# vllm-project/production-stack

Hardware: AMD Instinct MI355X
Metric: output_tokens_per_sec (higher is better)
Workload: dtype bfloat16; 1 GPU; multi-round-qa; model=llama-3-8b, users_per_gpu=320, rounds_per_conversation=10, max_model_len=8192, parallelism=dp1, prefix_caching=True, kv_cache_dtype=auto, quantization=none

## Files before the change

csrc/attention.hip:

```cpp
#include "ps_common.h"

template <int HEAD_DIM, int GQ, int BLOCK_SIZE, int NWAVES, int LOWREG,
          typename KVT>
__global__ __launch_bounds__(NWAVES * 64, LOWREG ? 3 : 1) void paged_attn_decode_kernel(
    unsigned short* __restrict__ out,
    float* __restrict__ ws_acc,
    float* __restrict__ ws_ml,
    const unsigned short* __restrict__ q,
    const KVT* __restrict__ k_cache,
    const KVT* __restrict__ v_cache,
    const int* __restrict__ block_tables,
    const int* __restrict__ seq_lens,
    int max_blocks, float scale, int KH, long q_stride, int window) {
  using KVTr = ps_kv_traits<KVT>;
  using kvec8 = typename KVTr::vec8;
  constexpr int D = HEAD_DIM;
  constexpr int LPG = D / 8;
  constexpr int TPW = 64 / LPG;
  static_assert(BLOCK_SIZE % TPW == 0, "block size must divide");

  const int seq = blockIdx.x;
  const int kvh = blockIdx.y;
  const int ctx = seq_lens[seq];
  const int wave = threadIdx.x >> 6;
  const int lane = threadIdx.x & 63;
  const int sg = lane / LPG;
  const int sl = lane % LPG;

  ps_bf16x8 qp[GQ];
  const unsigned short* qbase = q + (long)seq * q_stride + (long)kvh * GQ * D;
#pragma unroll
  for (int g = 0; g < GQ; g++)
    qp[g] = *(const ps_bf16x8*)(qbase + g * D + sl * 8);
  float qf[GQ][8];
  if constexpr (!LOWREG) {
#pragma unroll
    for (int g = 0; g < GQ; g++)
#pragma unroll
      for (int j = 0; j < 8; j++) qf[g][j] = ps_bf16_to_f32(qp[g][j]);
  }

  float m[GQ], l[GQ], acc[GQ][8];
#pragma unroll
  for (int g = 0; g < GQ; g++) {
    m[g] = PS_NEG_INF;
    l[g] = 0.f;
#pragma unroll
    for (int j = 0; j < 8; j++) acc[g][j] = 0.f;
  }

  const int nblocks = (ctx + BLOCK_SIZE - 1) / BLOCK_SIZE;
  const int win_lo = (window > 0 && ctx > window) ? ctx - window : 0;
  const int first_block = win_lo / BLOCK_SIZE;
  const int nsplit = gridDim.z;
  const int split = blockIdx.z;
  const int live_blocks = nblocks - first_block;
  const int per_split = (live_blocks + nsplit - 1) / nsplit;
  const int b_begin = first_block + split * per_split;
  const int b_end = min(nblocks, b_begin + per_split);
  const int* bt = block_tables + (long)seq * max_blocks;
  constexpr int TPB = BLOCK_SIZE / TPW;
  for (int b = b_begin + wave; b < b_end; b += NWAVES) {
    const long blk = bt[b];
    const KVT* kb = k_cache + ((blk * KH + kvh) * BLOCK_SIZE) * D;
    const KVT* vb = v_cache + ((blk * KH + kvh) * BLOCK_SIZE) * D;
    const int valid_tokens = min(BLOCK_SIZE, ctx - b * BLOCK_SIZE);
    float sc[GQ][TPB];
    kvec8 vv[TPB];
    if constexpr (LOWREG) {
#pragma unroll
      for (int g = 0; g < GQ; g++)
        asm volatile("" : "+v"(qp[g]));
    }
#pragma unroll
    for (int tt = 0; tt < TPB; tt++) {
      const int tok = tt * TPW + sg;
      const bool valid =
          tok < valid_tokens && b * BLOCK_SIZE + tok >= win_lo;
      kvec8 kv = *(const kvec8*)(kb + tok * D + sl * 8);
      if constexpr (!LOWREG)
        vv[tt] = *(const kvec8*)(vb + tok * D + sl * 8);
      float kf[8];
      KVTr::to_f32x8(kv, kf);
#pragma unroll
      for (int g = 0; g < GQ; g++) {
        float s = 0.f;
#pragma unroll
        for (int j = 0; j < 8; j++) {
          if constexpr (LOWREG)
            s += ps_bf16_to_f32(qp[g][j]) * kf[j];
          else
            s += qf[g][j] * kf[j];
        }
        s = ps_group_sum<LPG>(s) * scale;
        sc[g][tt] = valid ? s : PS_NEG_INF;
      }
    }
    if constexpr (LOWREG) {
#pragma unroll
      for (int tt = 0; tt < TPB; tt++)
        vv[tt] = *(const kvec8*)(vb + (tt * TPW + sg) * D + sl * 8);
    }
#pragma unroll
    for (int g = 0; g < GQ; g++) {
      float bmax = sc[g][0];
#pragma unroll
      for (int tt = 1; tt < TPB; tt++) bmax = fmaxf(bmax, sc[g][tt]);
      const float mnew = fmaxf(m[g], bmax);
      const float corr = __expf(m[g] - mnew);
      float p[TPB];
      float psum = 0.f;
#pragma unroll
      for (int tt = 0; tt < TPB; tt++) {
        p[tt] = sc[g][tt] > PS_NEG_INF ? __expf(sc[g][tt] - mnew) : 0.f;
        psum += p[tt];
// ... 32 lines not shown
  }

  __shared__ float sm[NWAVES][GQ];
  __shared__ float slse[NWAVES][GQ];
  __shared__ float sacc[NWAVES][GQ][D];
  if (sg == 0) {
#pragma unroll
    for (int g = 0; g < GQ; g++) {
      if (sl == 0) {
        sm[wave][g] = m[g];
        slse[wave][g] = l[g];
      }
#pragma unroll
      for (int j = 0; j < 8; j++) sacc[wave][g][sl * 8 + j] = acc[g][j];
    }
  }
  __syncthreads();
  if (wave == 0 && sg == 0) {
#pragma unroll
    for (int g = 0; g < GQ; g++) {
      float M = PS_NEG_INF, L = 0.f, A[8];
#pragma unroll
      for (int j = 0; j < 8; j++) A[j] = 0.f;
#pragma unroll
      for (int wv = 0; wv < NWAVES; wv++) {
        const float mw = sm[wv][g];
        const float mnew = fmaxf(M, mw);
        const float c1 = __expf(M - mnew);
        const float c2 = __expf(mw - mnew);
        L = L * c1 + slse[wv][g] * c2;
#pragma unroll
        for (int j = 0; j < 8; j++)
          A[j] = A[j] * c1 + sacc[wv][g][sl * 8 + j] * c2;
        M = mnew;
      }
      const long head = (long)seq * KH * GQ + (long)kvh * GQ + g;
      if (nsplit == 1) {
        const float inv = L > 0.f ? 1.f / L : 0.f;
        ps_bf16x8 ov;
#pragma unroll
        for (int j = 0; j < 8; j++) ov[j] = ps_f32_to_bf16(A[j] * inv);
        *(ps_bf16x8*)(out + head * D + sl * 8) = ov;
      } else {
        float* wa = ws_acc + (head * nsplit + split) * D + sl * 8;
#pragma unroll
        for (int j = 0; j < 8; j++) wa[j] = A[j];
        if (sl == 0) {
          float* wm = ws_ml + (head * nsplit + split) * 2;
          wm[0] = M;
          wm[1] = L;
        }
      }
    }
  }
}

template <int HEAD_DIM>
__global__ __launch_bounds__(64) void paged_attn_combine_kernel(
    unsigned short* __restrict__ out,
    const float* __restrict__ ws_acc,
    const float* __restrict__ ws_ml,
    int nsplit) {
  constexpr int D = HEAD_DIM;
  constexpr int LPG = D / 8;
  const long head = blockIdx.x;
  const int sl = threadIdx.x;
  if (sl >= LPG) return;
  float M = PS_NEG_INF, L = 0.f, A[8];
#pragma unroll
  for (int j = 0; j < 8; j++) A[j] = 0.f;
  for (int s = 0; s < nsplit; s++) {
    const float mw = ws_ml[(head * nsplit + s) * 2 + 0];
    const float lw = ws_ml[(head * nsplit + s) * 2 + 1];
    const float mnew = fmaxf(M, mw);
    const float c1 = __expf(M - mnew);
    const float c2 = __expf(mw - mnew);
    const float* wa = ws_acc + (head * nsplit + s) * D + sl * 8;
#pragma unroll
    for (int j = 0; j < 8; j++) A[j] = A[j] * c1 + wa[j] * c2;
    L = L * c1 + lw * c2;
    M = mnew;
  }
  const float inv = L > 0.f ? 1.f / L : 0.f;
  ps_bf16x8 ov;
#pragma unroll
  for (int j = 0; j < 8; j++) ov[j] = ps_f32_to_bf16(A[j] * inv);
  *(ps_bf16x8*)(out + head * D + sl * 8) = ov;
}

template <int HEAD_DIM, int BLOCK_SIZE>
__global__ __launch_bounds__(64) void paged_attn_prefill_kernel(
    unsigned short* __restrict__ out,
    const unsigned short* __restrict__ q,
    const unsigned short* __restrict__ k_cache,
    const unsigned short* __restrict__ v_cache,
    const int* __restrict__ block_tables,
    const int* __restrict__ token_seq,
    const int* __restrict__ token_pos,
    int max_blocks, float scale, int KH, int GQ, long q_stride,
    int window) {
  constexpr int D = HEAD_DIM;
  constexpr int LPG = D / 8;
  constexpr int TPW = 64 / LPG;

  const int tokid = blockIdx.x;
  const int qh = blockIdx.y;
// ... 123 lines not shown
    for (int j = 0; j < 8; j++) {
      const float f = ps_bf16_to_f32(xv[j]);
      if (f > best) {
        best = f;
        besti = i + j;
      }
    }
  }
  const int tail_start = (V / 8) * 8;
  for (int i = tail_start + threadIdx.x; i < V; i += blockDim.x) {
    const float f = ps_bf16_to_f32(row[i]);
    if (f > best) {
      best = f;
      besti = i;
    }
  }
#pragma unroll
  for (int off = 32; off > 0; off >>= 1) {
    const float ob = __shfl_xor(best, off, 64);
    const int oi = __shfl_xor(besti, off, 64);
    if (ob > best || (ob == best && oi < besti)) {
      best = ob;
      besti = oi;
    }
  }
  __shared__ float wbest[4];
  __shared__ int wbesti[4];
  const int wave = threadIdx.x >> 6;
  if ((threadIdx.x & 63) == 0) {
    wbest[wave] = best;
    wbesti[wave] = besti;
  }
  __syncthreads();
  if (threadIdx.x == 0) {
    for (int wv = 1; wv < (int)(blockDim.x >> 6); wv++) {
      if (wbest[wv] > wbest[0] ||
          (wbest[wv] == wbest[0] && wbesti[wv] < wbesti[0])) {
        wbest[0] = wbest[wv];
        wbesti[0] = wbesti[wv];
      }
    }
    out[r] = wbesti[0];
  }
}

extern "C" {

int ps_paged_attn_decode(void* out, void* ws_acc, void* ws_ml, const void* q,
                         const void* k_cache, const void* v_cache,
                         const void* block_tables, const void* seq_lens,
                         int num_seqs, int max_blocks, float scale, int KH,
                         int GQ, int head_dim, int block_size, int num_splits,
                         long q_stride, int variant, int kv_fp8,
                         int window, hipStream_t stream) {
  dim3 grid(num_seqs, KH, num_splits);
  constexpr int NW = 4;
  dim3 block(NW * 64);
#define PS_DECODE_T(HD, G, BS, LR, KVT)                                      \
  paged_attn_decode_kernel<HD, G, BS, NW, LR, KVT>                           \
      <<<grid, block, 0, stream>>>(                                          \
          (unsigned short*)out, (float*)ws_acc, (float*)ws_ml,               \
          (const unsigned short*)q, (const KVT*)k_cache,                     \
          (const KVT*)v_cache, (const int*)block_tables,                     \
          (const int*)seq_lens, max_blocks, scale, KH, q_stride, window)
#define PS_DISPATCH_DECODE(HD, G, BS)                                        \
  do {                                                                       \
    if (kv_fp8) {                                                            \
      if (variant == 1)                                                      \
        PS_DECODE_T(HD, G, BS, 1, unsigned char);                            \
      else                                                                   \
        PS_DECODE_T(HD, G, BS, 0, unsigned char);                            \
    } else {                                                                 \
      if (variant == 1)                                                      \
        PS_DECODE_T(HD, G, BS, 1, unsigned short);                           \
      else                                                                   \
        PS_DECODE_T(HD, G, BS, 0, unsigned short);                           \
    }                                                                        \
    if (num_splits > 1)                                                      \
      paged_attn_combine_kernel<HD>                                          \
          <<<dim3(num_seqs * KH * G), 64, 0, stream>>>(                      \
              (unsigned short*)out, (const float*)ws_acc,                    \
              (const float*)ws_ml, num_splits);                              \
  } while (0)
  if (head_dim == 128 && block_size == 16) {
    switch (GQ) {
      case 1: PS_DISPATCH_DECODE(128, 1, 16); return 0;
      case 2: PS_DISPATCH_DECODE(128, 2, 16); return 0;
      case 3: PS_DISPATCH_DECODE(128, 3, 16); return 0;
      case 4: PS_DISPATCH_DECODE(128, 4, 16); return 0;
      case 6: PS_DISPATCH_DECODE(128, 6, 16); return 0;
      case 7: PS_DISPATCH_DECODE(128, 7, 16); return 0;
      case 8: PS_DISPATCH_DECODE(128, 8, 16); return 0;
      default: return -1;
    }
  }
  if (head_dim == 64 && block_size == 16 && !kv_fp8) {
    switch (GQ) {
      case 1: PS_DISPATCH_DECODE(64, 1, 16); return 0;
      case 2: PS_DISPATCH_DECODE(64, 2, 16); return 0;
      case 4: PS_DISPATCH_DECODE(64, 4, 16); return 0;
      case 8: PS_DISPATCH_DECODE(64, 8, 16); return 0;
      default: return -1;
    }
  }
  return -1;
#undef PS_DECODE_T
#undef PS_DISPATCH_DECODE
}

int ps_paged_attn_prefill(void* out, const void* q, const void* k_cache,
                          const void* v_cache, const void* block_tables,
                          const void* token_seq, const void* token_pos,
                          int num_tokens, int num_q_heads, int max_blocks,
                          float scale, int KH, int GQ, int head_dim,
                          int block_size, long q_stride, int window,
                          hipStream_t stream) {
  dim3 grid(num_tokens, num_q_heads);
  dim3 block(64);
#define PS_DISPATCH_PREFILL(HD, BS)                                         \
  paged_attn_prefill_kernel<HD, BS><<<grid, block, 0, stream>>>(            \
      (unsigned short*)out, (const unsigned short*)q,                       \
      (const unsigned short*)k_cache, (const unsigned short*)v_cache,       \
      (const int*)block_tables, (const int*)token_seq,                      \
      (const int*)token_pos, max_blocks, scale, KH, GQ, q_stride, window)
  if (head_dim == 128 && block_size == 16) {
    PS_DISPATCH_PREFILL(128, 16);
    return 0;
  }
  if (head_dim == 64 && block_size == 16) {
    PS_DISPATCH_PREFILL(64, 16);
    return 0;
  }
  return -1;
#undef PS_DISPATCH_PREFILL
}

void ps_reshape_and_cache(const void* k, const void* v, void* k_cache,
                          void* v_cache, const void* slot_mapping, long T,
                          int KH, int HD, int BS, int kv_fp8,
                          hipStream_t stream) {
  const long total = T * (long)KH * HD / 8;
  const int block = 256;
  const long want = (total + block - 1) / block;
  const int grid = (int)(want < 2048 ? (want > 0 ? want : 1) : 2048);
  if (kv_fp8)
    reshape_and_cache_kernel<unsigned char><<<grid, block, 0, stream>>>(
        (const unsigned short*)k, (const unsigned short*)v,
        (unsigned char*)k_cache, (unsigned char*)v_cache,
        (const long*)slot_mapping, KH, HD, BS, total);
  else
    reshape_and_cache_kernel<unsigned short><<<grid, block, 0, stream>>>(
        (const unsigned short*)k, (const unsigned short*)v,
        (unsigned short*)k_cache, (unsigned short*)v_cache,
        (const long*)slot_mapping, KH, HD, BS, total);
}

void ps_greedy_sample(void* out, const void* logits, long R, int V,
                      hipStream_t stream) {
  greedy_sample_kernel<<<dim3((unsigned)R), 256, 0, stream>>>(
      (long*)out, (const unsigned short*)logits, V);
// ... 4 lines not shown
```

csrc/bindings.cpp:

```cpp
#include <hip/hip_runtime.h>
#include <torch/extension.h>

#include <c10/hip/HIPStream.h>

#include <algorithm>

extern "C" {
void ps_rms_norm(void* out, const void* x, const void* w, float eps, long T,
                 int D, hipStream_t stream);
void ps_fused_add_rms_norm(void* x, void* residual, const void* w, float eps,
                           long T, int D, hipStream_t stream);
void ps_rms_norm_fp8(void* out_q, void* out_scale, void* x, void* residual,
                     const void* w, float eps, long T, int D, int fused,
                     hipStream_t stream);
void ps_silu_and_mul_fp8(void* out_q, void* out_scale, const void* x, long T,
                         int D, hipStream_t stream);
void ps_silu_and_mul(void* out, const void* x, long T, int D,
                     hipStream_t stream);
void ps_rope(const void* positions, void* q, void* k, const void* cos_sin,
             long T, int QH, int KH, int HD, int ROT, hipStream_t stream);
void ps_fused_rope_cache(void* qkv, const void* positions, const void* cos_sin,
                         const void* slot_mapping, void* k_cache,
                         void* v_cache, long T, int QH, int KH, int HD,
                         int ROT, long qkv_stride, int BS, int kv_fp8,
                         hipStream_t stream);
int ps_paged_attn_decode(void* out, void* ws_acc, void* ws_ml, const void* q,
                         const void* k_cache, const void* v_cache,
                         const void* block_tables, const void* seq_lens,
                         int num_seqs, int max_blocks, float scale, int KH,
                         int GQ, int head_dim, int block_size, int num_splits,
                         long q_stride, int variant, int kv_fp8, int window,
                         hipStream_t stream);
int ps_prefill_mfma32_splits(int num_tiles, int KH, int GQ);
int ps_paged_attn_prefill_mfma32(void* out, void* ws_o, void* ws_ml,
                                 long q_tokens, const void* q,
                                 const void* k_cache, const void* v_cache,
                                 const void* block_tables,
                                 const void* tile_info, int num_tiles,
                                 int num_q_heads, int max_blocks,
                                 float scale, int KH, int GQ, int head_dim,
                                 long q_stride, int kv_fp8, int window,
                                 hipStream_t stream);
int ps_paged_attn_prefill_mfma(void* out, const void* q, const void* k_cache,
                               const void* v_cache, const void* block_tables,
                               const void* tile_info, int num_tiles,
                               int num_q_heads, int max_blocks, float scale,
                               int KH, int GQ, int head_dim, long q_stride,
                               int variant, int kv_fp8, int window, hipStream_t stream);
int ps_paged_attn_prefill(void* out, const void* q, const void* k_cache,
                          const void* v_cache, const void* block_tables,
                          const void* token_seq, const void* token_pos,
                          int num_tokens, int num_q_heads, int max_blocks,
                          float scale, int KH, int GQ, int head_dim,
                          int block_size, long q_stride, int window,
                          hipStream_t stream);
void ps_reshape_and_cache(const void* k, const void* v, void* k_cache,
                          void* v_cache, const void* slot_mapping, long T,
                          int KH, int HD, int BS, int kv_fp8,
                          hipStream_t stream);
void ps_greedy_sample(void* out, const void* logits, long R, int V,
                      hipStream_t stream);
void ps_kv_quant(void* out, void* scales, const void* in, long rows, int hd,
                 hipStream_t stream);
void ps_kv_dequant(void* out, const void* in, const void* scales, long rows,
                   int hd, hipStream_t stream);
int ps_skinny_gemm_splits(int M, int N, int K);
int ps_skinny_gemm(void* out_bf16, void* ws, const void* x, const void* w,
                   int M, int N, int K, long x_stride, hipStream_t stream);
int ps_gemm8p_splits(int M, int N, int K);
int ps_gemm8p(void* out_bf16, void* ws, const void* x, const void* w, int M,
              int N, int K, long x_stride, hipStream_t stream);
int ps_lora_bgmv(void* out, const void* x, const void* A, const void* B,
                 const void* scale, const void* idx, int T, int IN, int W,
                 int R, long out_stride, long x_stride, int col_off,
                 hipStream_t stream);
int ps_fused_moe_supported(int T, int top_k, int E, int H, int I);
int ps_fused_moe(void* out, void* offsets, void* sorted_pairs, void* act,
                 void* y, const void* x, const void* w_gate_up,
                 const void* w_down, const void* topk_ids, int ids_i64,
                 const void* topk_w, int T, int top_k, int E, int H, int I,
                 hipStream_t stream);
}

at::Tensor cachegen_encode(at::Tensor q);
at::Tensor cachegen_decode(at::Tensor blob, int64_t hd);
// ... 31 lines not shown
}

void rms_norm(at::Tensor out, at::Tensor x, at::Tensor w, double eps) {
  CHECK_GPU_BF16(out);
  CHECK_GPU_BF16(x);
  CHECK_GPU_BF16(w);
  const long T = x.numel() / x.size(-1);
  const int D = (int)x.size(-1);
  TORCH_CHECK(D % 8 == 0, "hidden dim must be a multiple of 8");
  ps_rms_norm(out.data_ptr(), x.data_ptr(), w.data_ptr(), (float)eps, T, D,
              current_stream());
}

void fused_add_rms_norm(at::Tensor x, at::Tensor residual, at::Tensor w,
                        double eps) {
  CHECK_GPU_BF16(x);
  CHECK_GPU_BF16(residual);
  CHECK_GPU_BF16(w);
  const long T = x.numel() / x.size(-1);
  const int D = (int)x.size(-1);
  TORCH_CHECK(D % 8 == 0, "hidden dim must be a multiple of 8");
  ps_fused_add_rms_norm(x.data_ptr(), residual.data_ptr(), w.data_ptr(),
                        (float)eps, T, D, current_stream());
}

void silu_and_mul(at::Tensor out, at::Tensor x) {
  CHECK_GPU_BF16(out);
  CHECK_GPU_BF16(x);
  const int D = (int)out.size(-1);
  TORCH_CHECK(x.size(-1) == 2 * D, "x last dim must be 2*out last dim");
  TORCH_CHECK(D % 8 == 0, "feature dim must be a multiple of 8");
  const long T = out.numel() / D;
  ps_silu_and_mul(out.data_ptr(), x.data_ptr(), T, D, current_stream());
}

void rotary_embedding(at::Tensor positions, at::Tensor q, at::Tensor k,
                      at::Tensor cos_sin, long head_dim) {
  CHECK_GPU_DTYPE(positions, at::kInt);
  CHECK_GPU_BF16(q);
  CHECK_GPU_BF16(k);
  CHECK_GPU_DTYPE(cos_sin, at::kFloat);
  const long T = positions.size(0);
  const int HD = (int)head_dim;
  const int ROT = (int)cos_sin.size(-1);
  const int QH = (int)(q.numel() / T / HD);
  const int KH = (int)(k.numel() / T / HD);
  ps_rope(positions.data_ptr(), q.data_ptr(), k.data_ptr(),
          cos_sin.data_ptr(), T, QH, KH, HD, ROT, current_stream());
}

void paged_attn_decode(at::Tensor out, at::Tensor q, at::Tensor k_cache,
                       at::Tensor v_cache, at::Tensor block_tables,
                       at::Tensor seq_lens, double scale, int64_t num_splits,
                       int64_t variant, int64_t window) {
  CHECK_GPU_BF16(out);
  const int kv_fp8 = cache_fp8(k_cache);
  cache_fp8(v_cache);
  CHECK_GPU_DTYPE(block_tables, at::kInt);
  CHECK_GPU_DTYPE(seq_lens, at::kInt);
  const int S = (int)q.size(0);
  const int QH = (int)q.size(1);
  const int HD = (int)q.size(2);
  const int KH = (int)k_cache.size(1);
  const int BS = (int)k_cache.size(2);
  TORCH_CHECK(QH % KH == 0, "GQA group mismatch");
  const int GQ = QH / KH;
  const int max_blocks = (int)block_tables.size(1);
  if (num_splits <= 0) {
    const int target = 2048;
    num_splits = std::min<int64_t>(
        32, std::max<int64_t>(1, target / std::max(1, S * KH)));
  }
  at::Tensor ws_acc, ws_ml;
  void *acc_p = nullptr, *ml_p = nullptr;
  if (num_splits > 1) {
    auto opts = q.options().dtype(at::kFloat);
    ws_acc = at::empty({(long)S * QH * num_splits * HD}, opts);
    ws_ml = at::empty({(long)S * QH * num_splits * 2}, opts);
    acc_p = ws_acc.data_ptr();
    ml_p = ws_ml.data_ptr();
  }
  int rc = ps_paged_attn_decode(
      out.data_ptr(), acc_p, ml_p, q.data_ptr(), k_cache.data_ptr(),
      v_cache.data_ptr(), block_tables.data_ptr(), seq_lens.data_ptr(), S,
      max_blocks, (float)scale, KH, GQ, HD, BS, (int)num_splits,
      q_row_stride(q, HD), (int)variant, kv_fp8, (int)window,
      current_stream());
  TORCH_CHECK(rc == 0, "unsupported decode config: head_dim=", HD,
              " block_size=", BS, " gqa=", GQ);
}

void paged_attn_prefill(at::Tensor out, at::Tensor q, at::Tensor k_cache,
                        at::Tensor v_cache, at::Tensor block_tables,
                        at::Tensor token_seq, at::Tensor token_pos,
                        double scale, int64_t window) {
  CHECK_GPU_BF16(out);
  CHECK_GPU_BF16(k_cache);
  CHECK_GPU_BF16(v_cache);
  CHECK_GPU_DTYPE(block_tables, at::kInt);
  CHECK_GPU_DTYPE(token_seq, at::kInt);
  CHECK_GPU_DTYPE(token_pos, at::kInt);
  const int T = (int)q.size(0);
  const int QH = (int)q.size(1);
  const int HD = (int)q.size(2);
  const int KH = (int)k_cache.size(1);
  const int BS = (int)k_cache.size(2);
  TORCH_CHECK(QH % KH == 0, "GQA group mismatch");
  const int GQ = QH / KH;
  const int max_blocks = (int)block_tables.size(1);
  int rc = ps_paged_attn_prefill(
      out.data_ptr(), q.data_ptr(), k_cache.data_ptr(), v_cache.data_ptr(),
      block_tables.data_ptr(), token_seq.data_ptr(), token_pos.data_ptr(), T,
      QH, max_blocks, (float)scale, KH, GQ, HD, BS, q_row_stride(q, HD),
      (int)window, current_stream());
  TORCH_CHECK(rc == 0, "unsupported prefill config: head_dim=", HD,
              " block_size=", BS);
}

void paged_attn_prefill_mfma(at::Tensor out, at::Tensor q,
                             at::Tensor k_cache, at::Tensor v_cache,
                             at::Tensor block_tables, at::Tensor tile_info,
                             double scale, int64_t variant, int64_t window) {
  CHECK_GPU_BF16(out);
  const int kv_fp8 = cache_fp8(k_cache);
  cache_fp8(v_cache);
  CHECK_GPU_DTYPE(block_tables, at::kInt);
  CHECK_GPU_DTYPE(tile_info, at::kInt);
  const int QH = (int)q.size(1);
  const int HD = (int)q.size(2);
  const int KH = (int)k_cache.size(1);
  TORCH_CHECK(QH % KH == 0, "GQA group mismatch");
  TORCH_CHECK(k_cache.size(2) == 16, "mfma prefill needs block_size 16");
  const int GQ = QH / KH;
  const int NT = (int)tile_info.size(0);
  int rc;
  if (variant == 5) {
    const int splits = ps_prefill_mfma32_splits(NT, KH, QH / KH);
    const long T = q.size(0);
    void *ws_o_p = nullptr, *ws_ml_p = nullptr;
    at::Tensor ws_o, ws_ml;
    if (splits > 1) {
      ws_o = at::empty({(long)splits * T * QH * HD},
// ... 214 lines not shown
  int rc = ps_fused_moe(
      out.data_ptr(), offsets.data_ptr(), sorted_pairs.data_ptr(),
      act.data_ptr(), y.data_ptr(), x.data_ptr(), experts_gate_up.data_ptr(),
      experts_down.data_ptr(), topk_ids.data_ptr(),
      topk_ids.scalar_type() == at::kLong ? 1 : 0, topk_w.data_ptr(), (int)T,
      (int)top_k, (int)E, (int)H, (int)I, current_stream());
  TORCH_CHECK(rc == 0, "fused_moe launch rejected");
}

void kv_quant(at::Tensor out, at::Tensor scales, at::Tensor in) {
  CHECK_GPU_DTYPE(out, at::kChar);
  CHECK_GPU_DTYPE(scales, at::kFloat);
  CHECK_GPU_BF16(in);
  const int hd = (int)in.size(-1);
  TORCH_CHECK(hd % 8 == 0, "row width must be multiple of 8");
  const long rows = in.numel() / hd;
  ps_kv_quant(out.data_ptr(), scales.data_ptr(), in.data_ptr(), rows, hd,
              current_stream());
}

void kv_dequant(at::Tensor out, at::Tensor in, at::Tensor scales) {
  CHECK_GPU_BF16(out);
  CHECK_GPU_DTYPE(in, at::kChar);
  CHECK_GPU_DTYPE(scales, at::kFloat);
  const int hd = (int)out.size(-1);
  const long rows = out.numel() / hd;
  ps_kv_dequant(out.data_ptr(), in.data_ptr(), scales.data_ptr(), rows, hd,
                current_stream());
}

void greedy_sample(at::Tensor out, at::Tensor logits) {
  CHECK_GPU_DTYPE(out, at::kLong);
  CHECK_GPU_BF16(logits);
  const long R = logits.size(0);
  const int V = (int)logits.size(1);
  ps_greedy_sample(out.data_ptr(), logits.data_ptr(), R, V, current_stream());
}

}

PYBIND11_MODULE(TORCH_EXTENSION_NAME, m) {
  m.def("rms_norm", &rms_norm, "RMSNorm (bf16)");
  m.def("fused_add_rms_norm", &fused_add_rms_norm,
        "Fused residual add + RMSNorm (bf16, in-place)");
  m.def("silu_and_mul", &silu_and_mul, "SiLU-and-mul (bf16)");
  m.def("rotary_embedding", &rotary_embedding,
        "Neox-style rotary embedding (bf16, in-place)");
  m.def("paged_attn_decode", &paged_attn_decode,
        "Paged attention, decode phase (bf16 KV, split-KV)",
        pybind11::arg("out"), pybind11::arg("q"), pybind11::arg("k_cache"),
        pybind11::arg("v_cache"), pybind11::arg("block_tables"),
        pybind11::arg("seq_lens"), pybind11::arg("scale"),
        pybind11::arg("num_splits") = 0, pybind11::arg("variant") = 0,
        pybind11::arg("window") = 0);
  m.def("paged_attn_prefill", &paged_attn_prefill,
        "Paged attention, chunked prefill (bf16 KV)");
  m.def("lora_bgmv", &lora_bgmv,
        "batched-grouped LoRA matvec (per-token adapter slots)");
  m.def("paged_attn_prefill_mfma", &paged_attn_prefill_mfma,
        "Paged attention, chunked prefill via MFMA tiles (head_dim 128)",
        pybind11::arg("out"), pybind11::arg("q"), pybind11::arg("k_cache"),
        pybind11::arg("v_cache"), pybind11::arg("block_tables"),
        pybind11::arg("tile_info"), pybind11::arg("scale"),
        pybind11::arg("variant") = 4, pybind11::arg("window") = 0);
  m.def("fused_rope_cache", &fused_rope_cache,
        "Fused RoPE + paged KV append on the packed qkv tensor");
  m.def("reshape_and_cache", &reshape_and_cache,
        "Append K/V for new tokens into the paged cache");
  m.def("greedy_sample", &greedy_sample, "Per-row argmax over vocab");
  m.def("kv_quant", &kv_quant, "Row-wise int8 KV quantization");
  m.def("rms_norm_fp8", &rms_norm_fp8,
        "RMSNorm (optionally fused residual add) emitting fp8 + row scales");
  m.def("silu_and_mul_fp8", &silu_and_mul_fp8,
        "SiLU-mul emitting fp8 + row scales");
  m.def("cachegen_encode", &cachegen_encode,
        "CacheGen-style adaptive range encode of int8 KV (CPU)");
  m.def("cachegen_decode", &cachegen_decode,
        "CacheGen-style range decode -> int8 (CPU)");
  m.def("gemm8p", &gemm8p,
        "8-phase deep-pipelined bf16 GEMM (out = x @ w.T)");
  m.def("skinny_gemm", &skinny_gemm,
        "Split-K MFMA GEMM for decode-shaped (M<=128) projections");
  m.def("gemm8p_splits", &ps_gemm8p_splits,
        "Split-K depth gemm8p picks for (M, N, K); -1 if unsupported");
  m.def("skinny_gemm_splits", &ps_skinny_gemm_splits,
        "Split-K depth skinny_gemm picks for (M, N, K); -1 if unsupported");
  m.def("kv_dequant", &kv_dequant, "Row-wise int8 KV dequantization");
  m.def("fused_moe", &fused_moe,
        "Grouped MoE expert MLP (align + gate_up/SiLU + down + combine)");
  m.def("fused_moe_supported", &fused_moe_supported,
        "Whether fused_moe accepts (T, top_k, E, H, I)");
}
```

production_stack_amd/engine/models/llama.py:

```python

from __future__ import annotations

import math
from typing import List, Optional

import torch
import torch.nn as nn
import torch.nn.functional as F

from production_stack_amd import ops
from production_stack_amd.ops import gemm_policy
from production_stack_amd.engine.config import ModelConfig
from production_stack_amd.parallel import state as pstate


class BatchMeta:

    def __init__(
        self,
        positions: torch.Tensor,
        slot_mapping: torch.Tensor,
        num_prefill_tokens: int,
        prefill_token_seq: Optional[torch.Tensor],
        prefill_token_pos: Optional[torch.Tensor],
        prefill_block_tables: Optional[torch.Tensor],
        num_decode_seqs: int,
        decode_seq_lens: Optional[torch.Tensor],
        decode_block_tables: Optional[torch.Tensor],
        prefill_tiles: Optional[torch.Tensor] = None,
        lora_groups=None,
        lora_idx: Optional[torch.Tensor] = None,
        mm_rows: Optional[torch.Tensor] = None,
        mm_embeds: Optional[torch.Tensor] = None,
    ) -> None:
        self.positions = positions
        self.slot_mapping = slot_mapping
        self.num_prefill_tokens = num_prefill_tokens
        self.prefill_token_seq = prefill_token_seq
        self.prefill_token_pos = prefill_token_pos
        self.prefill_block_tables = prefill_block_tables
        self.num_decode_seqs = num_decode_seqs
        self.decode_seq_lens = decode_seq_lens
        self.decode_block_tables = decode_block_tables
        self.prefill_tiles = prefill_tiles
        self.lora_groups = lora_groups or []
        self.lora_idx = lora_idx
        self.mm_rows = mm_rows
        self.mm_embeds = mm_embeds


def build_cos_sin_cache(
    head_dim: int, max_position: int, theta: float,
    rope_scaling=None,
) -> torch.Tensor:
    half = head_dim // 2
    inv = 1.0 / (
        theta ** (torch.arange(0, head_dim, 2, dtype=torch.float64) / head_dim)
    )
    if rope_scaling is not None:
        factor, low_f, high_f, orig_max = rope_scaling
        low_wl = orig_max / low_f
        high_wl = orig_max / high_f
        wavelen = 2 * math.pi / inv
        scaled = torch.where(wavelen > low_wl, inv / factor, inv)
        smooth = (orig_max / wavelen - low_f) / (high_f - low_f)
        mid = (1 - smooth) * (inv / factor) + smooth * inv
        in_band = (wavelen <= low_wl) & (wavelen >= high_wl)
        inv = torch.where(in_band, mid, scaled)
    t = torch.arange(max_position, dtype=torch.float64)
    freqs = torch.outer(t, inv)
    return torch.cat([freqs.cos(), freqs.sin()], dim=-1).float().contiguous()


class LlamaLayer(nn.Module):
    def __init__(self, cfg: ModelConfig, tp: int, layer_idx: int = 0) -> None:
        super().__init__()
        self.cfg = cfg
        self.layer_idx = layer_idx
        assert cfg.num_q_heads % tp == 0, "q heads must divide TP"
        assert cfg.num_kv_heads % tp == 0 or tp % cfg.num_kv_heads == 0
        self.q_heads = cfg.num_q_heads // tp
        self.kv_heads = max(cfg.num_kv_heads // tp, 1)
        self.head_dim = cfg.head_dim
        self.inter = cfg.intermediate_size // tp
        h = cfg.hidden_size
        qs = self.q_heads * self.head_dim
        kvs = self.kv_heads * self.head_dim
        self.qkv_proj = nn.Parameter(
            torch.empty(qs + 2 * kvs, h, dtype=torch.bfloat16)
        )
        self.o_proj = nn.Parameter(torch.empty(h, qs, dtype=torch.bfloat16))
        self.n_experts = cfg.num_experts
        self.top_k = cfg.num_experts_per_tok
        self.moe_backend = "loop"
        if self.n_experts:
            self.moe_gate = nn.Parameter(
                torch.empty(self.n_experts, h, dtype=torch.bfloat16)
            )
            self.experts_gate_up = nn.Parameter(
                torch.empty(self.n_experts, 2 * self.inter, h,
                            dtype=torch.bfloat16)
# ... 90 lines not shown
            q, k = ops.rotary_embedding(
                meta.positions, q, k, cos_sin, self.head_dim
            )
            ops.reshape_and_cache(
                k.view(T, self.kv_heads, self.head_dim),
                v.view(T, self.kv_heads, self.head_dim),
                k_cache,
                v_cache,
                meta.slot_mapping,
            )
            qh = q.view(T, self.q_heads, self.head_dim)
        outs: List[torch.Tensor] = []
        tp = meta.num_prefill_tokens
        if tp > 0:
            if (
                qh.is_cuda
                and self.head_dim == 128
                and meta.prefill_tiles is not None
            ):
                outs.append(
                    ops.paged_attn_prefill_mfma(
                        qh[:tp],
                        k_cache,
                        v_cache,
                        meta.prefill_block_tables,
                        meta.prefill_tiles,
                        self.scale,
                        self.window,
                    )
                )
            else:
                outs.append(
                    ops.paged_attn_prefill(
                        qh[:tp] if qh.is_cuda else qh[:tp].contiguous(),
                        k_cache,
                        v_cache,
                        meta.prefill_block_tables,
                        meta.prefill_token_seq,
                        meta.prefill_token_pos,
                        self.scale,
                        self.window,
                    )
                )
        if meta.num_decode_seqs > 0:
            outs.append(
                ops.paged_attn_decode(
                    qh[tp:] if qh.is_cuda else qh[tp:].contiguous(),
                    k_cache,
                    v_cache,
                    meta.decode_block_tables,
                    meta.decode_seq_lens,
                    self.scale,
                    self.window,
                )
            )
        attn = torch.cat(outs, dim=0) if len(outs) > 1 else outs[0]
        if getattr(self, "fp8_w", None) is not None:
            attn_out = ops.fp8_linear(attn.reshape(T, qs),
                                      *self.fp8_w["o"])
        else:
            attn_out = gemm_policy.linear(attn.view(T, qs), self.o_proj)
        if slots is not None and meta.lora_idx is not None:
            slots.apply("o", self.layer_idx, attn_out,
                        attn.reshape(T, qs), meta.lora_idx)
        elif meta.lora_groups:
            apply_lora_slice(
                attn_out, attn.view(T, qs), meta.lora_groups,
                self.layer_idx, "o",
            )
        attn_out = pstate.tp_all_reduce(attn_out)

        if self.n_experts:
            hidden, residual = ops.fused_add_rms_norm(
                attn_out, residual, self.post_attn_norm, cfg.rms_norm_eps
            )
            mlp_out = self._moe_forward(hidden)
            mlp_out = pstate.tp_all_reduce(mlp_out)
            return mlp_out, residual
        if fuse_q:
            xq, sx = ops.rms_norm_fp8(
                attn_out, self.post_attn_norm, cfg.rms_norm_eps,
                residual=residual)
            hidden = attn_out
            gate_up = ops.fp8_linear_rowwise(xq, sx, *fp8["gate_up"])
        else:
            hidden, residual = ops.fused_add_rms_norm(
                attn_out, residual, self.post_attn_norm, cfg.rms_norm_eps
            )
            if fp8 is not None:
                gate_up = ops.fp8_linear(hidden, *fp8["gate_up"])
            else:
                gate_up = gemm_policy.linear(hidden, self.gate_up_proj)
        if slots is not None and meta.lora_idx is not None:
            slots.apply("gate", self.layer_idx, gate_up, hidden,
                        meta.lora_idx)
            slots.apply("up", self.layer_idx, gate_up, hidden,
                        meta.lora_idx)
        elif meta.lora_groups:
            apply_lora_slice(
                gate_up, hidden, meta.lora_groups, self.layer_idx,
                "gate", 0, self.inter,
            )
            apply_lora_slice(
                gate_up, hidden, meta.lora_groups, self.layer_idx,
                "up", self.inter, self.inter,
            )
# ... 113 lines not shown
        for layer in self.layers:
            fp8_w = {}
            proj_names = [("qkv", "qkv_proj"), ("o", "o_proj")]
            if not layer.n_experts:
                proj_names += [("gate_up", "gate_up_proj"),
                               ("down", "down_proj")]
            for key, pname in proj_names:
                w = getattr(layer, pname)
                if (w.is_cuda
                        and ops.fp8_rowwise_supported(w.device)):
                    w_q, scale = ops.fp8_quantize_weight_rowwise(w.data)
                else:
                    w_q, scale = ops.fp8_quantize_weight(w.data)
                fp8_w[key] = (w_q, scale.to(w.device))
                w.data = torch.empty(0, dtype=torch.bfloat16,
                                     device=w.device)
            layer.fp8_w = fp8_w

    @property
    def kv_heads(self) -> int:
        return max(self.cfg.num_kv_heads // self.tp, 1)

    @property
    def num_local_layers(self) -> int:
        return self.layer_end - self.layer_start

    def kv_bytes_per_block(self, block_size: int) -> int:
        return (
            2
            * self.kv_heads
            * block_size
            * self.cfg.head_dim
            * 2
            * self.num_local_layers
        )

    @torch.no_grad()
    def forward(
        self,
        token_ids: torch.Tensor,
        meta: BatchMeta,
        kv_caches: List[tuple],
        residual: Optional[torch.Tensor] = None,
    ) -> torch.Tensor:
        if self.is_first:
            hidden = F.embedding(token_ids, self.embed)
            if meta.mm_rows is not None:
                hidden = hidden.index_copy(
                    0, meta.mm_rows, meta.mm_embeds.to(hidden.dtype)
                )
            residual = None
        else:
            hidden = token_ids
        for layer, cache in zip(self.layers, kv_caches):
            hidden, residual = layer(
                hidden, residual, meta, cache, self.cos_sin
            )
        if not self.is_last:
            return torch.stack([hidden, residual])
        hidden, _ = ops.fused_add_rms_norm(
            hidden, residual, self.final_norm, self.cfg.rms_norm_eps
        )
        return hidden

    @torch.no_grad()
    def compute_logits(self, hidden: torch.Tensor) -> torch.Tensor:
        return F.linear(hidden, self.lm_head)
```

production_stack_amd/ops/__init__.py:

```python

from __future__ import annotations

import os

import torch

from production_stack_amd.ops import reference

try:
    from production_stack_amd import _C
except ImportError:
    _C = None

HAVE_EXT = _C is not None


def _require_ext() -> None:
    if _C is None:
        raise RuntimeError(
            "production_stack_amd._C HIP extension is not built; run "
            "`PYTORCH_ROCM_ARCH=gfx950 python setup.py build_ext --inplace`. "
            "Refusing to fall back to eager PyTorch on GPU."
        )


def rms_norm(x: torch.Tensor, w: torch.Tensor, eps: float) -> torch.Tensor:
    if x.is_cuda:
        _require_ext()
        out = torch.empty_like(x)
        _C.rms_norm(out, x, w, eps)
        return out
    return reference.rms_norm(x, w, eps)


def fused_add_rms_norm(
    x: torch.Tensor, residual: torch.Tensor, w: torch.Tensor, eps: float
) -> tuple[torch.Tensor, torch.Tensor]:
    if x.is_cuda:
        _require_ext()
        _C.fused_add_rms_norm(x, residual, w, eps)
        return x, residual
    normed, summed = reference.fused_add_rms_norm(x, residual, w, eps)
    return normed, summed


def silu_and_mul(x: torch.Tensor) -> torch.Tensor:
    if x.is_cuda:
        _require_ext()
        d = x.shape[-1] // 2
        out = torch.empty(x.shape[:-1] + (d,), dtype=x.dtype, device=x.device)
        _C.silu_and_mul(out, x)
        return out
    return reference.silu_and_mul(x)


def rotary_embedding(
    positions: torch.Tensor,
    q: torch.Tensor,
    k: torch.Tensor,
    cos_sin: torch.Tensor,
    head_dim: int,
) -> tuple[torch.Tensor, torch.Tensor]:
    if q.is_cuda:
        _require_ext()
        _C.rotary_embedding(positions, q, k, cos_sin, head_dim)
        return q, k
    return reference.rotary_embedding(positions, q, k, cos_sin, head_dim)


def fused_rope_cache(
    qkv: torch.Tensor,
    positions: torch.Tensor,
    cos_sin: torch.Tensor,
    slot_mapping: torch.Tensor,
    k_cache: torch.Tensor,
    v_cache: torch.Tensor,
    q_heads: int,
    head_dim: int,
) -> None:
    _require_ext()
    _C.fused_rope_cache(
        qkv, positions, cos_sin, slot_mapping, k_cache, v_cache, q_heads,
        head_dim,
    )


def reshape_and_cache(
    k: torch.Tensor,
    v: torch.Tensor,
    k_cache: torch.Tensor,
    v_cache: torch.Tensor,
    slot_mapping: torch.Tensor,
) -> None:
    if k_cache.is_cuda:
        _require_ext()
        _C.reshape_and_cache(
            k.view(k.shape[0], -1), v.view(v.shape[0], -1), k_cache, v_cache,
            slot_mapping,
        )
        return
    reference.reshape_and_cache(k, v, k_cache, v_cache, slot_mapping)


def paged_attn_decode(
    q: torch.Tensor,
    k_cache: torch.Tensor,
    v_cache: torch.Tensor,
    block_tables: torch.Tensor,
    seq_lens: torch.Tensor,
    scale: float,
    window: int = 0,
) -> torch.Tensor:
    if q.is_cuda:
        _require_ext()
        out = torch.empty(q.shape, dtype=q.dtype, device=q.device)
        _C.paged_attn_decode(
            out, q, k_cache, v_cache, block_tables, seq_lens, scale, 0, 1,
            window
        )
        return out
    return reference.paged_attn_decode(
        q, k_cache, v_cache, block_tables, seq_lens, scale, window
    )


def paged_attn_prefill(
    q: torch.Tensor,
    k_cache: torch.Tensor,
    v_cache: torch.Tensor,
    block_tables: torch.Tensor,
    token_seq: torch.Tensor,
    token_pos: torch.Tensor,
    scale: float,
    window: int = 0,
) -> torch.Tensor:
    if q.is_cuda:
        _require_ext()
        out = torch.empty(q.shape, dtype=q.dtype, device=q.device)
        _C.paged_attn_prefill(
            out, q, k_cache, v_cache, block_tables, token_seq, token_pos,
            scale, window
        )
        return out
    return reference.paged_attn_prefill(
        q, k_cache, v_cache, block_tables, token_seq, token_pos, scale,
        window
    )


PREFILL_VARIANT = int(os.environ.get("PS_PREFILL_VARIANT", "5"))


def prefill_tile_rows(num_q_heads: int, num_kv_heads: int) -> int:
    if PREFILL_VARIANT != 5:
        return 64
    gq = max(1, num_q_heads // max(1, num_kv_heads))
    gqw = 1
    while gqw < 4 and gq % (gqw * 2) == 0:
        gqw *= 2
    return 32 * (8 // gqw)


def paged_attn_prefill_mfma(
    q: torch.Tensor,
    k_cache: torch.Tensor,
    v_cache: torch.Tensor,
    block_tables: torch.Tensor,
    tile_info: torch.Tensor,
    scale: float,
    window: int = 0,
    variant: int = None,
) -> torch.Tensor:
    _require_ext()
    out = torch.empty(q.shape, dtype=q.dtype, device=q.device)
    v = PREFILL_VARIANT if variant is None else variant
    _C.paged_attn_prefill_mfma(
# ... 217 lines not shown
```

Before: 5623 tokens/s.

## Schedule decode attention longest-first and add pipelined block-table prefetch variant

```diff
diff --git a/csrc/attention.hip b/csrc/attention.hip
--- a/csrc/attention.hip
+++ b/csrc/attention.hip
@@ -1,7 +1,7 @@
 #include "ps_common.h"
 
 template <int HEAD_DIM, int GQ, int BLOCK_SIZE, int NWAVES, int LOWREG,
-          typename KVT>
+          typename KVT, int PIPE = 0>
 __global__ __launch_bounds__(NWAVES * 64, LOWREG ? 3 : 1) void paged_attn_decode_kernel(
     unsigned short* __restrict__ out,
     float* __restrict__ ws_acc,
@@ -11,6 +11,7 @@
     const KVT* __restrict__ v_cache,
     const int* __restrict__ block_tables,
     const int* __restrict__ seq_lens,
+    const int* __restrict__ order,
     int max_blocks, float scale, int KH, long q_stride, int window) {
   using KVTr = ps_kv_traits<KVT>;
   using kvec8 = typename KVTr::vec8;
@@ -18,8 +19,10 @@
   constexpr int LPG = D / 8;
   constexpr int TPW = 64 / LPG;
   static_assert(BLOCK_SIZE % TPW == 0, "block size must divide");
-
-  const int seq = blockIdx.x;
+  static_assert(!PIPE || LOWREG, "the pipelined loop is a LOWREG variant");
+
+  const int seq = order ? order[blockIdx.x] : blockIdx.x;
+  if ((unsigned)seq >= gridDim.x) return;
   const int kvh = blockIdx.y;
   const int ctx = seq_lens[seq];
   const int wave = threadIdx.x >> 6;
@@ -60,7 +63,74 @@
   const int b_end = min(nblocks, b_begin + per_split);
   const int* bt = block_tables + (long)seq * max_blocks;
   constexpr int TPB = BLOCK_SIZE / TPW;
-  for (int b = b_begin + wave; b < b_end; b += NWAVES) {
+  if constexpr (PIPE != 0) {
+    int b = b_begin + wave;
+    if (b < b_end) {
+      const int lane_off = sg * D + sl * 8;
+      long blk = __builtin_amdgcn_readfirstlane(bt[b]);
+      for (; b < b_end; b += NWAVES) {
+        const long blk_next = __builtin_amdgcn_readfirstlane(
+            bt[b + NWAVES < b_end ? b + NWAVES : b]);
+        const KVT* kb = k_cache + ((blk * KH + kvh) * BLOCK_SIZE) * D;
+        const KVT* vb = v_cache + ((blk * KH + kvh) * BLOCK_SIZE) * D;
+        const int valid_tokens = min(BLOCK_SIZE, ctx - b * BLOCK_SIZE);
+        float sc[GQ][TPB];
+        kvec8 vv[TPB];
+#pragma unroll
+        for (int g = 0; g < GQ; g++)
+          asm volatile("" : "+v"(qp[g]));
+#pragma unroll
+        for (int tt = 0; tt < TPB; tt++) {
+          const int tok = tt * TPW + sg;
+          const bool valid =
+              tok < valid_tokens && b * BLOCK_SIZE + tok >= win_lo;
+          kvec8 kv = *(const kvec8*)(kb + tt * TPW * D + lane_off);
+          float kf[8];
+          KVTr::to_f32x8(kv, kf);
+#pragma unroll
+          for (int g = 0; g < GQ; g++) {
+            float s = 0.f;
+#pragma unroll
+            for (int j = 0; j < 8; j++)
+              s += ps_bf16_to_f32(qp[g][j]) * kf[j];
+            s = ps_group_sum<LPG>(s) * scale;
+            sc[g][tt] = valid ? s : PS_NEG_INF;
+          }
+        }
+#pragma unroll
+        for (int tt = 0; tt < TPB; tt++)
+          vv[tt] = *(const kvec8*)(vb + tt * TPW * D + lane_off);
+#pragma unroll
+        for (int g = 0; g < GQ; g++) {
+          float bmax = sc[g][0];
+#pragma unroll
+          for (int tt = 1; tt < TPB; tt++) bmax = fmaxf(bmax, sc[g][tt]);
+          const float mnew = fmaxf(m[g], bmax);
+          const float corr = __expf(m[g] - mnew);
+          float p[TPB];
+          float psum = 0.f;
+#pragma unroll
+          for (int tt = 0; tt < TPB; tt++) {
+            p[tt] = sc[g][tt] > PS_NEG_INF ? __expf(sc[g][tt] - mnew) : 0.f;
+            psum += p[tt];
+          }
+          l[g] = l[g] * corr + psum;
+#pragma unroll
+          for (int j = 0; j < 8; j++) acc[g][j] *= corr;
+#pragma unroll
+          for (int tt = 0; tt < TPB; tt++) {
+            float vf[8];
+            KVTr::to_f32x8(vv[tt], vf);
+#pragma unroll
+            for (int j = 0; j < 8; j++) acc[g][j] += p[tt] * vf[j];
+          }
+          m[g] = mnew;
+        }
+        blk = blk_next;
+      }
+    }
+  }
+  for (int b = PIPE ? b_end : b_begin + wave; b < b_end; b += NWAVES) {
     const long blk = bt[b];
     const KVT* kb = k_cache + ((blk * KH + kvh) * BLOCK_SIZE) * D;
     const KVT* vb = v_cache + ((blk * KH + kvh) * BLOCK_SIZE) * D;
@@ -199,6 +269,25 @@
         }
       }
     }
+  }
+}
+
+#define PS_DECODE_ORDER_MAX 4096
+__global__ __launch_bounds__(1024) void decode_order_kernel(
+    int* __restrict__ order,
+    const int* __restrict__ seq_lens,
+    int S) {
+  __shared__ int lens[PS_DECODE_ORDER_MAX];
+  for (int i = threadIdx.x; i < S; i += blockDim.x) lens[i] = seq_lens[i];
+  __syncthreads();
+  for (int i = threadIdx.x; i < S; i += blockDim.x) {
+    const int li = lens[i];
+    int rank = 0;
+    for (int j = 0; j < S; j++) {
+      const int lj = lens[j];
+      rank += (lj > li || (lj == li && j < i)) ? 1 : 0;
+    }
+    order[rank] = i;
   }
 }
 
@@ -428,30 +517,35 @@
                          int num_seqs, int max_blocks, float scale, int KH,
                          int GQ, int head_dim, int block_size, int num_splits,
                          long q_stride, int variant, int kv_fp8,
-                         int window, hipStream_t stream) {
+                         int window, const void* order,
+                         hipStream_t stream) {
+  if (variant < 0 || variant > 2) return -1;
   dim3 grid(num_seqs, KH, num_splits);
   constexpr int NW = 4;
   dim3 block(NW * 64);
-#define PS_DECODE_T(HD, G, BS, LR, KVT)                                      \
-  paged_attn_decode_kernel<HD, G, BS, NW, LR, KVT>                           \
+#define PS_DECODE_T(HD, G, BS, LR, KVT, PIPE)                                \
+  paged_attn_decode_kernel<HD, G, BS, NW, LR, KVT, PIPE>                     \
       <<<grid, block, 0, stream>>>(                                          \
           (unsigned short*)out, (float*)ws_acc, (float*)ws_ml,               \
           (const unsigned short*)q, (const KVT*)k_cache,                     \
           (const KVT*)v_cache, (const int*)block_tables,                     \
-          (const int*)seq_lens, max_blocks, scale, KH, q_stride, window)
+          (const int*)seq_lens, (const int*)order, max_blocks, scale, KH,    \
+          q_stride, window)
+#define PS_DECODE_V(HD, G, BS, KVT)                                          \
+  do {                                                                       \
+    if (variant == 2)                                                        \
+      PS_DECODE_T(HD, G, BS, 1, KVT, 1);                                     \
+    else if (variant == 1)                                                   \
+      PS_DECODE_T(HD, G, BS, 1, KVT, 0);                                     \
+    else                                                                     \
+      PS_DECODE_T(HD, G, BS, 0, KVT, 0);                                     \
+  } while (0)
 #define PS_DISPATCH_DECODE(HD, G, BS)                                        \
   do {                                                                       \
-    if (kv_fp8) {                                                            \
-      if (variant == 1)                                                      \
-        PS_DECODE_T(HD, G, BS, 1, unsigned char);                            \
-      else                                                                   \
-        PS_DECODE_T(HD, G, BS, 0, unsigned char);                            \
-    } else {                                                                 \
-      if (variant == 1)                                                      \
-        PS_DECODE_T(HD, G, BS, 1, unsigned short);                           \
-      else                                                                   \
-        PS_DECODE_T(HD, G, BS, 0, unsigned short);                           \
-    }                                                                        \
+    if (kv_fp8)                                                              \
+      PS_DECODE_V(HD, G, BS, unsigned char);                                 \
+    else                                                                     \
+      PS_DECODE_V(HD, G, BS, unsigned short);                                \
     if (num_splits > 1)                                                      \
       paged_attn_combine_kernel<HD>                                          \
           <<<dim3(num_seqs * KH * G), 64, 0, stream>>>(                      \
@@ -481,7 +575,17 @@
   }
   return -1;
 #undef PS_DECODE_T
+#undef PS_DECODE_V
 #undef PS_DISPATCH_DECODE
+}
+
+int ps_decode_order(void* order, const void* seq_lens, int S,
+                    hipStream_t stream) {
+  if (S < 1 || S > PS_DECODE_ORDER_MAX) return -1;
+  const int threads = S <= 256 ? 256 : 1024;
+  decode_order_kernel<<<1, threads, 0, stream>>>((int*)order,
+                                                 (const int*)seq_lens, S);
+  return 0;
 }
 
 int ps_paged_attn_prefill(void* out, const void* q, const void* k_cache,
diff --git a/csrc/bindings.cpp b/csrc/bindings.cpp
--- a/csrc/bindings.cpp
+++ b/csrc/bindings.cpp
@@ -30,7 +30,9 @@
                          int num_seqs, int max_blocks, float scale, int KH,
                          int GQ, int head_dim, int block_size, int num_splits,
                          long q_stride, int variant, int kv_fp8, int window,
-                         hipStream_t stream);
+                         const void* order, hipStream_t stream);
+int ps_decode_order(void* order, const void* seq_lens, int S,
+                    hipStream_t stream);
 int ps_prefill_mfma32_splits(int num_tiles, int KH, int GQ);
 int ps_paged_attn_prefill_mfma32(void* out, void* ws_o, void* ws_ml,
                                  long q_tokens, const void* q,
@@ -168,13 +170,21 @@
 void paged_attn_decode(at::Tensor out, at::Tensor q, at::Tensor k_cache,
                        at::Tensor v_cache, at::Tensor block_tables,
                        at::Tensor seq_lens, double scale, int64_t num_splits,
-                       int64_t variant, int64_t window) {
+                       int64_t variant, int64_t window,
+                       c10::optional<at::Tensor> order) {
   CHECK_GPU_BF16(out);
   const int kv_fp8 = cache_fp8(k_cache);
   cache_fp8(v_cache);
   CHECK_GPU_DTYPE(block_tables, at::kInt);
   CHECK_GPU_DTYPE(seq_lens, at::kInt);
   const int S = (int)q.size(0);
+  const void* order_p = nullptr;
+  if (order.has_value()) {
+    const at::Tensor& order_t = *order;
+    CHECK_GPU_DTYPE(order_t, at::kInt);
+    TORCH_CHECK(order_t.numel() == S, "order must have one entry per seq");
+    order_p = order_t.data_ptr();
+  }
   const int QH = (int)q.size(1);
   const int HD = (int)q.size(2);
   const int KH = (int)k_cache.size(1);
@@ -200,10 +210,18 @@
       out.data_ptr(), acc_p, ml_p, q.data_ptr(), k_cache.data_ptr(),
       v_cache.data_ptr(), block_tables.data_ptr(), seq_lens.data_ptr(), S,
       max_blocks, (float)scale, KH, GQ, HD, BS, (int)num_splits,
-      q_row_stride(q, HD), (int)variant, kv_fp8, (int)window,
+      q_row_stride(q, HD), (int)variant, kv_fp8, (int)window, order_p,
       current_stream());
   TORCH_CHECK(rc == 0, "unsupported decode config: head_dim=", HD,
-              " block_size=", BS, " gqa=", GQ);
+              " block_size=", BS, " gqa=", GQ, " variant=", variant);
+}
+
+bool decode_order(at::Tensor order, at::Tensor seq_lens) {
+  CHECK_GPU_DTYPE(order, at::kInt);
+  CHECK_GPU_DTYPE(seq_lens, at::kInt);
+  TORCH_CHECK(order.numel() == seq_lens.numel(), "order/seq_lens size");
+  return ps_decode_order(order.data_ptr(), seq_lens.data_ptr(),
+                         (int)seq_lens.numel(), current_stream()) == 0;
 }
 
 void paged_attn_prefill(at::Tensor out, at::Tensor q, at::Tensor k_cache,
@@ -524,7 +542,10 @@
         pybind11::arg("v_cache"), pybind11::arg("block_tables"),
         pybind11::arg("seq_lens"), pybind11::arg("scale"),
         pybind11::arg("num_splits") = 0, pybind11::arg("variant") = 0,
-        pybind11::arg("window") = 0);
+        pybind11::arg("window") = 0,
+        pybind11::arg("order") = pybind11::none());
+  m.def("decode_order", &decode_order,
+        "Longest-first sequence order for paged_attn_decode");
   m.def("paged_attn_prefill", &paged_attn_prefill,
         "Paged attention, chunked prefill (bf16 KV)");
   m.def("lora_bgmv", &lora_bgmv,
diff --git a/production_stack_amd/engine/models/llama.py b/production_stack_amd/engine/models/llama.py
--- a/production_stack_amd/engine/models/llama.py
+++ b/production_stack_amd/engine/models/llama.py
@@ -47,6 +47,15 @@
         self.lora_idx = lora_idx
         self.mm_rows = mm_rows
         self.mm_embeds = mm_embeds
+        self.decode_order: Optional[torch.Tensor] = None
+
+
+def _decode_order_wanted(meta: BatchMeta) -> bool:
+    return (
+        ops.DECODE_ORDER
+        and meta.num_decode_seqs > 0
+        and meta.decode_seq_lens.is_cuda
+    )
 
 
 def build_cos_sin_cache(
@@ -243,6 +252,7 @@
                     meta.decode_seq_lens,
                     self.scale,
                     self.window,
+                    meta.decode_order,
                 )
             )
         attn = torch.cat(outs, dim=0) if len(outs) > 1 else outs[0]
@@ -462,6 +472,9 @@
             residual = None
         else:
             hidden = token_ids
+        meta.decode_order = None
+        if _decode_order_wanted(meta):
+            meta.decode_order = ops.decode_order(meta.decode_seq_lens)
         for layer, cache in zip(self.layers, kv_caches):
             hidden, residual = layer(
                 hidden, residual, meta, cache, self.cos_sin
diff --git a/production_stack_amd/ops/__init__.py b/production_stack_amd/ops/__init__.py
--- a/production_stack_amd/ops/__init__.py
+++ b/production_stack_amd/ops/__init__.py
@@ -2,6 +2,7 @@
 from __future__ import annotations
 
 import os
+from typing import Optional
 
 import torch
 
@@ -102,6 +103,10 @@
     reference.reshape_and_cache(k, v, k_cache, v_cache, slot_mapping)
 
 
+DECODE_VARIANT = int(os.environ.get("PS_DECODE_VARIANT", "2"))
+DECODE_ORDER = os.environ.get("PS_DECODE_ORDER", "1") != "0"
+
+
 def paged_attn_decode(
     q: torch.Tensor,
     k_cache: torch.Tensor,
@@ -110,18 +115,29 @@
     seq_lens: torch.Tensor,
     scale: float,
     window: int = 0,
+    order: Optional[torch.Tensor] = None,
 ) -> torch.Tensor:
     if q.is_cuda:
         _require_ext()
         out = torch.empty(q.shape, dtype=q.dtype, device=q.device)
         _C.paged_attn_decode(
-            out, q, k_cache, v_cache, block_tables, seq_lens, scale, 0, 1,
-            window
+            out, q, k_cache, v_cache, block_tables, seq_lens, scale, 0,
+            DECODE_VARIANT, window, order
         )
         return out
     return reference.paged_attn_decode(
         q, k_cache, v_cache, block_tables, seq_lens, scale, window
     )
+
+
+def decode_order(seq_lens: torch.Tensor) -> Optional[torch.Tensor]:
+    if seq_lens.is_cuda:
+        _require_ext()
+        order = torch.empty_like(seq_lens)
+        if not _C.decode_order(order, seq_lens):
+            return None
+        return order
+    return torch.argsort(-seq_lens, stable=True).int()
 
 
 def paged_attn_prefill(
```

Result: faster. 5791 tokens/s, median of 6 (+3.0%).
